# KeyuWu-CS/MonoHair

Measured on AMD Instinct MI355X. Metric: PMVO iterations/sec (60x1080p views, 256^3 volume), higher is better.
Workload: dtype f32

## Files before the change

monohair_amd/csrc/mh_key_blocks.h:

```cpp
template <int NI, int KN>
__device__ __forceinline__ void mh_key_block4(unsigned (&ke)[KN], unsigned (&ko)[KN], const float2 (&g)[4],
                                              const float (&DX)[KN], const float (&DY)[KN], int ib) {
    static_assert(NI >= 1 && NI <= 4 && NI <= KN, "mh_key_block4: 1..4 items");
    float a[NI], b[NI], c[NI];
    if constexpr (NI == 4) {
        asm volatile(
            "v_mul_f32_e32 %[a0], %[t0x], %[x0]\n\t"
            "v_mul_f32_e32 %[a1], %[t0x], %[x1]\n\t"
            "v_mul_f32_e32 %[a2], %[t0x], %[x2]\n\t"
            "v_mul_f32_e32 %[a3], %[t0x], %[x3]\n\t"
            "v_mul_f32_e32 %[b0], %[t0y], %[y0]\n\t"
            "v_mul_f32_e32 %[b1], %[t0y], %[y1]\n\t"
            "v_mul_f32_e32 %[b2], %[t0y], %[y2]\n\t"
            "v_mul_f32_e32 %[b3], %[t0y], %[y3]\n\t"
            "v_mul_f32_e32 %[c0], %[t2x], %[x0]\n\t"
            "v_mul_f32_e32 %[c1], %[t2x], %[x1]\n\t"
            "v_mul_f32_e32 %[c2], %[t2x], %[x2]\n\t"
            "v_mul_f32_e32 %[c3], %[t2x], %[x3]\n\t"
            "v_add_f32_e32 %[a0], %[a0], %[b0]\n\t"
            "v_add_f32_e32 %[a1], %[a1], %[b1]\n\t"
            "v_add_f32_e32 %[a2], %[a2], %[b2]\n\t"
            "v_add_f32_e32 %[a3], %[a3], %[b3]\n\t"
            "v_mul_f32_e32 %[b0], %[t2y], %[y0]\n\t"
            "v_mul_f32_e32 %[b1], %[t2y], %[y1]\n\t"
// ... 172 lines not shown
            "v_mul_f32_e32 %[b0], %[t1y], %[y0]\n\t"
            "v_mul_f32_e32 %[b1], %[t1y], %[y1]\n\t"
            "v_mul_f32_e32 %[c0], %[t3x], %[x0]\n\t"
            "v_mul_f32_e32 %[c1], %[t3x], %[x1]\n\t"
            "v_add_f32_e32 %[a0], %[a0], %[b0]\n\t"
            "v_add_f32_e32 %[a1], %[a1], %[b1]\n\t"
            "v_mul_f32_e32 %[b0], %[t3y], %[y0]\n\t"
            "v_mul_f32_e32 %[b1], %[t3y], %[y1]\n\t"
            "v_sub_f32_e64 %[a0], %[cc], |%[a0]|\n\t"
            "v_sub_f32_e64 %[a1], %[cc], |%[a1]|\n\t"
            "v_add_f32_e32 %[c0], %[c0], %[b0]\n\t"
            "v_add_f32_e32 %[c1], %[c1], %[b1]\n\t"
            "v_lshl_or_b32 %[a0], %[a0], 5, %[i0]\n\t"
            "v_lshl_or_b32 %[a1], %[a1], 5, %[i0]\n\t"
            "v_sub_f32_e64 %[c0], %[cc], |%[c0]|\n\t"
            "v_sub_f32_e64 %[c1], %[cc], |%[c1]|\n\t"
            "v_lshl_or_b32 %[c0], %[c0], 5, %[i1]\n\t"
            "v_lshl_or_b32 %[c1], %[c1], 5, %[i1]\n\t"
            "v_min3_u32 %[o0], %[o0], %[a0], %[c0]\n\t"
            "v_min3_u32 %[o1], %[o1], %[a1], %[c1]"
            : [e0] "+v"(ke[0]), [e1] "+v"(ke[1]), [o0] "+v"(ko[0]), [o1] "+v"(ko[1]), [a0] "=&v"(a[0]), [a1] "=&v"(a[1]), [b0] "=&v"(b[0]), [b1] "=&v"(b[1]), [c0] "=&v"(c[0]), [c1] "=&v"(c[1])
            : [t0x] "v"(g[0].x), [t0y] "v"(g[0].y), [t1x] "v"(g[1].x), [t1y] "v"(g[1].y), [t2x] "v"(g[2].x), [t2y] "v"(g[2].y), [t3x] "v"(g[3].x), [t3y] "v"(g[3].y), [x0] "v"(DX[0]), [y0] "v"(DY[0]), [x1] "v"(DX[1]), [y1] "v"(DY[1]), [cc] "s"(MH_KEY_C), [i0] "s"(ib), [i1] "s"(ib + 1)
            : "memory");
    }
    else if constexpr (NI == 1) {
        asm volatile(
            "v_mul_f32_e32 %[a0], %[t0x], %[x0]\n\t"
            "v_mul_f32_e32 %[b0], %[t0y], %[y0]\n\t"
            "v_mul_f32_e32 %[c0], %[t2x], %[x0]\n\t"
            "v_add_f32_e32 %[a0], %[a0], %[b0]\n\t"
            "v_mul_f32_e32 %[b0], %[t2y], %[y0]\n\t"
            "v_sub_f32_e64 %[a0], %[cc], |%[a0]|\n\t"
            "v_add_f32_e32 %[c0], %[c0], %[b0]\n\t"
            "v_lshl_or_b32 %[a0], %[a0], 5, %[i0]\n\t"
            "v_sub_f32_e64 %[c0], %[cc], |%[c0]|\n\t"
            "v_lshl_or_b32 %[c0], %[c0], 5, %[i1]\n\t"
            "v_min3_u32 %[e0], %[e0], %[a0], %[c0]\n\t"
            "v_mul_f32_e32 %[a0], %[t1x], %[x0]\n\t"
            "v_mul_f32_e32 %[b0], %[t1y], %[y0]\n\t"
            "v_mul_f32_e32 %[c0], %[t3x], %[x0]\n\t"
            "v_add_f32_e32 %[a0], %[a0], %[b0]\n\t"
            "v_mul_f32_e32 %[b0], %[t3y], %[y0]\n\t"
            "v_sub_f32_e64 %[a0], %[cc], |%[a0]|\n\t"
            "v_add_f32_e32 %[c0], %[c0], %[b0]\n\t"
            "v_lshl_or_b32 %[a0], %[a0], 5, %[i0]\n\t"
            "v_sub_f32_e64 %[c0], %[cc], |%[c0]|\n\t"
            "v_lshl_or_b32 %[c0], %[c0], 5, %[i1]\n\t"
            "v_min3_u32 %[o0], %[o0], %[a0], %[c0]"
            : [e0] "+v"(ke[0]), [o0] "+v"(ko[0]), [a0] "=&v"(a[0]), [b0] "=&v"(b[0]), [c0] "=&v"(c[0])
            : [t0x] "v"(g[0].x), [t0y] "v"(g[0].y), [t1x] "v"(g[1].x), [t1y] "v"(g[1].y), [t2x] "v"(g[2].x), [t2y] "v"(g[2].y), [t3x] "v"(g[3].x), [t3y] "v"(g[3].y), [x0] "v"(DX[0]), [y0] "v"(DY[0]), [cc] "s"(MH_KEY_C), [i0] "s"(ib), [i1] "s"(ib + 1)
            : "memory");
    }
}
```

monohair_amd/csrc/pmvo_search.hip:

```cpp
#include "mh_search_common.h"
#include "../../include/mh_pmvo_lab.h"

__device__ __forceinline__ void mh_sample_next(const float *__restrict__ cam, float X0, float X1, float X2,
                                               float ori_r, float ori_c, float Hf, float Wf, float off, float &S0,
                                               float &S1, float &S2, int forms) {
    alignas(16) float rec[16];
    mh_sample_rank(cam, X0, X1, X2, ori_r, ori_c, Hf, Wf, rec, forms);
    mh_sample_item(reinterpret_cast<const float4 *>(rec), off, S0, S1, S2);
}

__device__ __forceinline__ float mh_one_minus_abs(float x) {
    float r;
    asm("v_sub_f32_e64 %0, 1.0, |%1|" : "=v"(r) : "v"(x));
    return r;
}

template <int K, int T>
__global__ __launch_bounds__(T) void mh_search_kernel(MhViews vw, const float *__restrict__ offs, int S, int nrank,
                                                      int rank_step, const float *__restrict__ pts, int N, int P1,
                                                      float thr, const float *__restrict__ ori_c,
                                                      const int32_t *__restrict__ base_idx,
                                                      const float *__restrict__ base_val,
                                                      const float4 *__restrict__ taps, float *__restrict__ line_ori,
                                                      float *__restrict__ min_loss, uint8_t *__restrict__ high_conf,
// ... 182 lines not shown
        asm("v_cmp_lt_f32_e64 %[m0], %[l0], %[a0]\n\t"
            "v_cmp_lt_f32_e64 %[m1], %[l1], %[a1]\n\t"
            "v_cmp_lt_f32_e64 %[m2], %[l2], %[a2]\n\t"
            "v_cmp_lt_f32_e64 %[m3], %[l3], %[a3]\n\t"
            "v_cndmask_b32_e64 %[a0], %[a0], %[l0], %[m0]\n\t"
            "v_cndmask_b32_e64 %[a1], %[a1], %[l1], %[m1]\n\t"
            "v_cndmask_b32_e64 %[a2], %[a2], %[l2], %[m2]\n\t"
            "v_cndmask_b32_e64 %[a3], %[a3], %[l3], %[m3]\n\t"
            "v_cndmask_b32_e64 %[b0], %[b0], %[cf], %[m0]\n\t"
            "v_cndmask_b32_e64 %[b1], %[b1], %[cf], %[m1]\n\t"
            "v_cndmask_b32_e64 %[b2], %[b2], %[cf], %[m2]\n\t"
            "v_cndmask_b32_e64 %[b3], %[b3], %[cf], %[m3]"
            : [a0] "+v"(ML[0]), [a1] "+v"(ML[1]), [a2] "+v"(ML[2]), [a3] "+v"(ML[3]), [b0] "+v"(BC[0]),
              [b1] "+v"(BC[1]), [b2] "+v"(BC[2]), [b3] "+v"(BC[3]), [m0] "=&s"(m0), [m1] "=&s"(m1), [m2] "=&s"(m2),
              [m3] "=&s"(m3)
            : [l0] "v"(l[0]), [l1] "v"(l[1]), [l2] "v"(l[2]), [l3] "v"(l[3]), [cf] "v"(cf));
    } else if constexpr (KA == 3) {
        unsigned long long m0, m1, m2;
        asm("v_cmp_lt_f32_e64 %[m0], %[l0], %[a0]\n\t"
            "v_cmp_lt_f32_e64 %[m1], %[l1], %[a1]\n\t"
            "v_cmp_lt_f32_e64 %[m2], %[l2], %[a2]\n\t"
            "v_cndmask_b32_e64 %[a0], %[a0], %[l0], %[m0]\n\t"
            "v_cndmask_b32_e64 %[a1], %[a1], %[l1], %[m1]\n\t"
            "v_cndmask_b32_e64 %[a2], %[a2], %[l2], %[m2]\n\t"
            "v_cndmask_b32_e64 %[b0], %[b0], %[cf], %[m0]\n\t"
            "v_cndmask_b32_e64 %[b1], %[b1], %[cf], %[m1]\n\t"
            "v_cndmask_b32_e64 %[b2], %[b2], %[cf], %[m2]"
            : [a0] "+v"(ML[0]), [a1] "+v"(ML[1]), [a2] "+v"(ML[2]), [b0] "+v"(BC[0]), [b1] "+v"(BC[1]),
              [b2] "+v"(BC[2]), [m0] "=&s"(m0), [m1] "=&s"(m1), [m2] "=&s"(m2)
            : [l0] "v"(l[0]), [l1] "v"(l[1]), [l2] "v"(l[2]), [cf] "v"(cf));
    } else if constexpr (KA == 2) {
        unsigned long long m0, m1;
        asm("v_cmp_lt_f32_e64 %[m0], %[l0], %[a0]\n\t"
            "v_cmp_lt_f32_e64 %[m1], %[l1], %[a1]\n\t"
            "s_nop 0\n\t"
            "v_cndmask_b32_e64 %[a0], %[a0], %[l0], %[m0]\n\t"
            "v_cndmask_b32_e64 %[a1], %[a1], %[l1], %[m1]\n\t"
            "v_cndmask_b32_e64 %[b0], %[b0], %[cf], %[m0]\n\t"
            "v_cndmask_b32_e64 %[b1], %[b1], %[cf], %[m1]"
            : [a0] "+v"(ML[0]), [a1] "+v"(ML[1]), [b0] "+v"(BC[0]), [b1] "+v"(BC[1]), [m0] "=&s"(m0), [m1] "=&s"(m1)
            : [l0] "v"(l[0]), [l1] "v"(l[1]), [cf] "v"(cf));
    } else {
#pragma unroll
        for (int j = 0; j < KA; ++j) {
            const bool upd = l[j] < ML[j];
            ML[j] = upd ? l[j] : ML[j];
            BC[j] = upd ? cf : BC[j];
        }
    }
}

#define MH_KEY_C 1.00006103515625f
#define MH_KEY_E 6.103515625e-05f
#define MH_KEY_BAD 0xF0000000u
#ifndef MH_KEY_MIN_TAPS
#define MH_KEY_MIN_TAPS 10
#endif
#define MH_KEY_PAD 4
template <bool BIGP>
__device__ __forceinline__ int mh_key_walked(int c) {
    return (c - (BIGP ? 0 : 1) + MH_KEY_PAD - 1) & ~(MH_KEY_PAD - 1);
}
template <bool BIGP>
__device__ __forceinline__ int mh_key_staged(int c) {
    const int w = mh_key_walked<BIGP>(c);
    return w > c ? w : c;
}
__device__ unsigned long long mh_key_stats_dev[4];
extern "C" int mh_debug_key_stats(unsigned long long *out, int reset) {
    if (hipMemcpyFromSymbol(out, HIP_SYMBOL(mh_key_stats_dev), sizeof(unsigned long long) * 4) != hipSuccess) return -1;
    if (reset) {
        const unsigned long long z[4] = {0, 0, 0, 0};
        if (hipMemcpyToSymbol(HIP_SYMBOL(mh_key_stats_dev), z, sizeof(z)) != hipSuccess) return -1;
    }
    return 0;
}
#define MH_KEY_COUNT_ALWAYS(i) do { if ((tid & 63) == 0) atomicAdd(&mh_key_stats_dev[i], 1ull); } while (0)
#ifdef MH_KEY_STATS
#define MH_KEY_COUNT(i) MH_KEY_COUNT_ALWAYS(i)
#else
#define MH_KEY_COUNT(i) do { } while (0)
#endif
__device__ __forceinline__ unsigned mh_tap_key(float cs, int idx) {
    float t;
    unsigned k;
    asm("v_sub_f32_e64 %0, %2, |%1|" : "=v"(t) : "v"(cs), "s"(MH_KEY_C));
    asm("v_lshl_or_b32 %0, %1, 5, %2" : "=v"(k) : "v"(t), "s"(idx));
    return k;
}
__device__ __forceinline__ unsigned mh_min3u(unsigned a, unsigned b, unsigned c) {
    unsigned r;
    asm("v_min3_u32 %0, %1, %2, %3" : "=v"(r) : "v"(a), "v"(b), "v"(c));
    return r;
}

#include "mh_key_blocks.h"

#define MH_S3_GRP 4
#ifndef MH_S3_WAVES
#define MH_S3_WAVES 5
#endif
#ifndef MH_S3_WAVES_SELECT
#define MH_S3_WAVES_SELECT MH_S3_WAVES
#endif
#define MH_S3_CAP 1280

template <bool BIG>
struct MhCascS {
    float a0 = 0.0f, a1 = 0.0f, a2 = 0.0f;
    __device__ __forceinline__ void flush(int v) {
        a1 = a1 + a0;
        a0 = 0.0f;
        if constexpr (BIG) {
            if ((v & 0xF0) == 0) {
                a2 = a2 + a1;
                a1 = 0.0f;
            }
        }
    }
    __device__ __forceinline__ float done() const { return BIG ? (a0 + a1) + a2 : (a0 + a1); }
};

__device__ __forceinline__ int mh_wave_prefix_sum(int x) {
#define MH_DPP_ADD(CTRL, ROWS) x += __builtin_amdgcn_update_dpp(0, x, CTRL, ROWS, 0xF, false)
    MH_DPP_ADD(0x111, 0xF);
    MH_DPP_ADD(0x112, 0xF);
    MH_DPP_ADD(0x114, 0xF);
    MH_DPP_ADD(0x118, 0xF);
    MH_DPP_ADD(0x142, 0xA);
    MH_DPP_ADD(0x143, 0xC);
#undef MH_DPP_ADD
    return x;
}

__device__ __forceinline__ int mh_lane_now() {
    int lane;
    asm volatile("v_mbcnt_lo_u32_b32 %0, -1, 0\n\tv_mbcnt_hi_u32_b32 %0, -1, %0" : "=v"(lane));
    return lane;
}

// ... 186 lines not shown
                DX[2 * jp] = dx.x;
                DX[2 * jp + 1] = dx.y;
                DY[2 * jp] = dy.x;
                DY[2 * jp + 1] = dy.y;
            }
            if constexpr (KA & 1) {
                float row, col;
                mh_pixel_of_fast1(cam, X0[KA - 1], X1[KA - 1], X2[KA - 1], Hf, Wf, row, col);
                mh_unit2_fast1(row - hdr.z, col - hdr.w, DX[KA - 1], DY[KA - 1]);
            }
        }
        constexpr int GRP = MH_S3_GRP;
        auto select_body = [&]() {
#pragma unroll
            for (int j = 0; j < KA; ++j) {
                ML[j] = mh_one_minus_abs(mh_vadd(mh_vmul(t0.x, DX[j]), mh_vmul(t0.y, DY[j])));
                BC[j] = t0.z;
            }
            auto process = [&](const float4 (&g)[GRP], int t) {
#pragma unroll
                for (int u = 0; u < GRP; ++u) {
                    if (t + u < ntap) {
                        const float4 tp = g[u];
                        float l[KN];
#pragma unroll
                        for (int j = 0; j < KA; ++j)
                            l[j] = mh_one_minus_abs(mh_vadd(mh_vmul(tp.x, DX[j]), mh_vmul(tp.y, DY[j])));
                        mh_tap_update<KN>(ML, BC, l, tp.z);
                    }
                }
            };
            float4 ga[GRP], gb[GRP];
#pragma unroll
            for (int u = 0; u < GRP; ++u) ga[u] = rec[2 + u];
            for (int t = 1; t < ntap;) {
#pragma unroll
                for (int u = 0; u < GRP; ++u) gb[u] = rec[1 + t + GRP + u];
                process(ga, t);
                t += GRP;
                if (t >= ntap) break;
#pragma unroll
                for (int u = 0; u < GRP; ++u) ga[u] = rec[1 + t + GRP + u];
                process(gb, t);
                t += GRP;
            }
        };
        __builtin_amdgcn_s_setprio(0);
        if constexpr (!KEYS) {
            select_body();
        } else {
            bool again = (ntap <= MH_KEY_MIN_TAPS) || !(t0.x == t0.x && t0.y == t0.y);
            MH_KEY_COUNT(0);
            if (again) MH_KEY_COUNT(1);
            if (!again) {
                const int ntp = mh_key_walked<BIGP>(ntap);
                unsigned ke[KN], ko[KN];
                const unsigned rec1 = (unsigned)(size_t)(const __attribute__((address_space(3))) float4 *)(rec + 1);
                auto process = [&](const float2 (&g)[GRP], int t) {
                    const int ib = (t & 63) >> 1;
                    static_assert(MH_KEY_PAD == 4 && GRP == 4, "the key block takes four taps");
                    if constexpr (KM > 0) mh_key_block4<KM, KN>(ke, ko, g, DX, DY, ib);
                };
                auto group = [&](int ta, int tb) {
                    const float2 *__restrict__ t2 = reinterpret_cast<const float2 *>(rec + 1);
                    float2 ga[GRP], gb[GRP];
#pragma unroll
                    for (int u = 0; u < GRP; ++u) ga[u] = t2[2 * (ta + u)];
                    if constexpr (BIGP || KM == 0) {
#pragma unroll
                        for (int j = 0; j < KN; ++j) ke[j] = ko[j] = 0xFFFFFFFFu;
                    } else {
                        const int is = ntap - 1;
                        const float2 ts = t2[2 * is];
                        const bool even = (is & 1) == 0;
#pragma unroll
                        for (int j = 0; j < KM; ++j) {
                            const unsigned k = mh_tap_key(mh_vadd(mh_vmul(ts.x, DX[j]), mh_vmul(ts.y, DY[j])), is >> 1);
                            ke[j] = even ? k : 0xFFFFFFFFu;
                            ko[j] = even ? 0xFFFFFFFFu : k;
                        }
                    }
                    for (int t = ta; t < tb;) {
#pragma unroll
                        for (int u = 0; u < GRP; ++u) gb[u] = t2[2 * (t + GRP + u)];
                        process(ga, t);
                        t += GRP;
                        if (t >= tb) break;
#pragma unroll
                        for (int u = 0; u < GRP; ++u) ga[u] = t2[2 * (t + GRP + u)];
                        process(gb, t);
                        t += GRP;
                    }
                };
                unsigned best[KN], badr[KN];
                auto winner = [&](int ta, bool first) {
#pragma unroll
                    for (int j = 0; j < KM; ++j) {
                        const bool odd = ko[j] < ke[j];
                        const unsigned kb = odd ? ko[j] : ke[j];
                        const unsigned ad = rec1 + 16u * (unsigned)ta + ((kb & 31u) << 5) + (odd ? 16u : 0u);
                        const bool take = first || kb < (best[j] & ~31u);
                        best[j] = take ? kb : best[j];
                        badr[j] = take ? ad : badr[j];
                    }
                };
                if constexpr (!BIGP) {
                    group(0, ntp);
                    winner(0, true);
                } else {
                    group(0, ntp < 64 ? ntp : 64);
                    winner(0, true);
                    for (int ta = 64; ta < ntp; ta += 64) {
                        group(ta, ntp < ta + 64 ? ntp : ta + 64);
                        winner(ta, false);
                    }
                }
                unsigned worst = best[0];
#pragma unroll
                for (int j = 1; j < KM; ++j) worst = max(worst, best[j]);
                const bool bad = worst >= MH_KEY_BAD;
#pragma unroll
                for (int j = 0; j < KM; ++j) {
                    BC[j] = *reinterpret_cast<const __attribute__((address_space(3))) float *>((size_t)(badr[j] + 8u));
                    ML[j] = __uint_as_float(__builtin_amdgcn_alignbit(7u, best[j], 5u)) - MH_KEY_E;
                }
                again = __ballot(bad) != 0ull;
                if (again) MH_KEY_COUNT_ALWAYS(2);
            }
            if (again) select_body();
        }
        __builtin_amdgcn_s_setprio(1);
#pragma unroll
        for (int j = 0; j < KA; ++j) {
            const float w = BC[j];
            num[j].a0 = num[j].a0 + ML[j] * w;
            den[j].a0 = den[j].a0 + w;
            cnt[j] += (w > 0.0f) ? 1 : 0;
        }
    };
    const int lane = tid & 63, wave = __builtin_amdgcn_readfirstlane(tid >> 6);
    int c = c_first, pre = pre_first;
    for (int vb = 0; vb < V; vb += 64) {
        if (vb) {
            const int vv = vb + lane;
            c = (vv < V) ? (int)vcnt[(size_t)vv * N + n] : 0;
            pre = mh_wave_prefix_sum(mh_list_records<KEYS, BIGP>(c));
        }
        bool staged = vb == 0;
        unsigned long long todo = __ballot(c != 0);
        int base = 0;
        if constexpr (LEFT) {
            if (left && lane == 0) lf.vis[vb >> 6] = todo;
        }
        while (todo) {
            const unsigned long long take = todo & __ballot(pre - base <= MH_S3_CAP);
            if (!staged) {
                mh_stage_batch<T, KEYS, BIGP>(taps, s_taps, vb, n, N, P1, c, pre, base, take, wave);
                __syncthreads();
            }
            staged = false;
            if constexpr (KA > 0) {
                unsigned long long m = take;
                while (m) {
                    const int b = (int)__builtin_ctzll(m);
                    m &= m - 1;
                    flush_upto(vb + b);
                    const int cb = __builtin_amdgcn_readlane(c, b);
                    const int L = mh_list_records<KEYS, BIGP>(cb);
                    const int off = __builtin_amdgcn_readlane(pre, b) - L - base;
                    one_view(vb + b, s_taps + off, cb);
                }
            }
            if constexpr (LEFT) {
// ... 412 lines not shown
```

Measured before the change: 1812.

## Use block-index keys with a single min accumulator in the small-tap key search

After: 1833 (median of 6 runs). 1.2% higher.

```diff
diff --git a/monohair_amd/csrc/mh_key_blocks.h b/monohair_amd/csrc/mh_key_blocks.h
--- a/monohair_amd/csrc/mh_key_blocks.h
+++ b/monohair_amd/csrc/mh_key_blocks.h
@@ -248,3 +248,458 @@
             : "memory");
     }
 }
+
+template <int NI, int KN, bool FOLD>
+__device__ __forceinline__ void mh_key_blockm4(unsigned (&acc)[KN], unsigned (&kk)[KN], const float2 (&g)[4],
+                                               const float (&DX)[KN], const float (&DY)[KN], int ib) {
+    static_assert(NI >= 1 && NI <= 4 && NI <= KN, "mh_key_blockm4: 1..4 items");
+    constexpr int NW = NI < 2 ? NI : 2;
+    float a[NW], b[NW], c[NW];
+    [[maybe_unused]] float d[NW];
+    if constexpr (NI == 4) {
+        if constexpr (FOLD) {
+            asm volatile(
+                "v_mul_f32_e32 %[a0], %[t0x], %[x0]\n\t"
+                "v_mul_f32_e32 %[a1], %[t0x], %[x1]\n\t"
+                "v_mul_f32_e32 %[b0], %[t0y], %[y0]\n\t"
+                "v_mul_f32_e32 %[b1], %[t0y], %[y1]\n\t"
+                "v_mul_f32_e32 %[c0], %[t2x], %[x0]\n\t"
+                "v_mul_f32_e32 %[c1], %[t2x], %[x1]\n\t"
+                "v_add_f32_e32 %[a0], %[a0], %[b0]\n\t"
+                "v_add_f32_e32 %[a1], %[a1], %[b1]\n\t"
+                "v_mul_f32_e32 %[b0], %[t2y], %[y0]\n\t"
+                "v_mul_f32_e32 %[b1], %[t2y], %[y1]\n\t"
+                "v_sub_f32_e64 %[a0], %[cc], |%[a0]|\n\t"
+                "v_sub_f32_e64 %[a1], %[cc], |%[a1]|\n\t"
+                "v_add_f32_e32 %[c0], %[c0], %[b0]\n\t"
+                "v_add_f32_e32 %[c1], %[c1], %[b1]\n\t"
+                "v_mul_f32_e32 %[d0], %[t1x], %[x0]\n\t"
+                "v_mul_f32_e32 %[d1], %[t1x], %[x1]\n\t"
+                "v_sub_f32_e64 %[c0], %[cc], |%[c0]|\n\t"
+                "v_sub_f32_e64 %[c1], %[cc], |%[c1]|\n\t"
+                "v_mul_f32_e32 %[b0], %[t1y], %[y0]\n\t"
+                "v_mul_f32_e32 %[b1], %[t1y], %[y1]\n\t"
+                "v_min_u32_e32 %[a0], %[a0], %[c0]\n\t"
+                "v_min_u32_e32 %[a1], %[a1], %[c1]\n\t"
+                "v_mul_f32_e32 %[c0], %[t3x], %[x0]\n\t"
+                "v_mul_f32_e32 %[c1], %[t3x], %[x1]\n\t"
+                "v_add_f32_e32 %[d0], %[d0], %[b0]\n\t"
+                "v_add_f32_e32 %[d1], %[d1], %[b1]\n\t"
+                "v_mul_f32_e32 %[b0], %[t3y], %[y0]\n\t"
+                "v_mul_f32_e32 %[b1], %[t3y], %[y1]\n\t"
+                "v_sub_f32_e64 %[d0], %[cc], |%[d0]|\n\t"
+                "v_sub_f32_e64 %[d1], %[cc], |%[d1]|\n\t"
+                "v_add_f32_e32 %[c0], %[c0], %[b0]\n\t"
+                "v_add_f32_e32 %[c1], %[c1], %[b1]\n\t"
+                "v_sub_f32_e64 %[c0], %[cc], |%[c0]|\n\t"
+                "v_sub_f32_e64 %[c1], %[cc], |%[c1]|\n\t"
+                "v_min3_u32 %[a0], %[a0], %[d0], %[c0]\n\t"
+                "v_min3_u32 %[a1], %[a1], %[d1], %[c1]\n\t"
+                "v_lshl_or_b32 %[a0], %[a0], 4, %[ib]\n\t"
+                "v_lshl_or_b32 %[a1], %[a1], 4, %[ib]\n\t"
+                "v_min3_u32 %[m0], %[m0], %[k0], %[a0]\n\t"
+                "v_min3_u32 %[m1], %[m1], %[k1], %[a1]\n\t"
+                "v_mul_f32_e32 %[a0], %[t0x], %[x2]\n\t"
+                "v_mul_f32_e32 %[a1], %[t0x], %[x3]\n\t"
+                "v_mul_f32_e32 %[b0], %[t0y], %[y2]\n\t"
+                "v_mul_f32_e32 %[b1], %[t0y], %[y3]\n\t"
+                "v_mul_f32_e32 %[c0], %[t2x], %[x2]\n\t"
+                "v_mul_f32_e32 %[c1], %[t2x], %[x3]\n\t"
+                "v_add_f32_e32 %[a0], %[a0], %[b0]\n\t"
+                "v_add_f32_e32 %[a1], %[a1], %[b1]\n\t"
+                "v_mul_f32_e32 %[b0], %[t2y], %[y2]\n\t"
+                "v_mul_f32_e32 %[b1], %[t2y], %[y3]\n\t"
+                "v_sub_f32_e64 %[a0], %[cc], |%[a0]|\n\t"
+                "v_sub_f32_e64 %[a1], %[cc], |%[a1]|\n\t"
+                "v_add_f32_e32 %[c0], %[c0], %[b0]\n\t"
+                "v_add_f32_e32 %[c1], %[c1], %[b1]\n\t"
+                "v_mul_f32_e32 %[d0], %[t1x], %[x2]\n\t"
+                "v_mul_f32_e32 %[d1], %[t1x], %[x3]\n\t"
+                "v_sub_f32_e64 %[c0], %[cc], |%[c0]|\n\t"
+                "v_sub_f32_e64 %[c1], %[cc], |%[c1]|\n\t"
+                "v_mul_f32_e32 %[b0], %[t1y], %[y2]\n\t"
+                "v_mul_f32_e32 %[b1], %[t1y], %[y3]\n\t"
+                "v_min_u32_e32 %[a0], %[a0], %[c0]\n\t"
+                "v_min_u32_e32 %[a1], %[a1], %[c1]\n\t"
+                "v_mul_f32_e32 %[c0], %[t3x], %[x2]\n\t"
+                "v_mul_f32_e32 %[c1], %[t3x], %[x3]\n\t"
+                "v_add_f32_e32 %[d0], %[d0], %[b0]\n\t"
+                "v_add_f32_e32 %[d1], %[d1], %[b1]\n\t"
+                "v_mul_f32_e32 %[b0], %[t3y], %[y2]\n\t"
+                "v_mul_f32_e32 %[b1], %[t3y], %[y3]\n\t"
+                "v_sub_f32_e64 %[d0], %[cc], |%[d0]|\n\t"
+                "v_sub_f32_e64 %[d1], %[cc], |%[d1]|\n\t"
+                "v_add_f32_e32 %[c0], %[c0], %[b0]\n\t"
+                "v_add_f32_e32 %[c1], %[c1], %[b1]\n\t"
+                "v_sub_f32_e64 %[c0], %[cc], |%[c0]|\n\t"
+                "v_sub_f32_e64 %[c1], %[cc], |%[c1]|\n\t"
+                "v_min3_u32 %[a0], %[a0], %[d0], %[c0]\n\t"
+                "v_min3_u32 %[a1], %[a1], %[d1], %[c1]\n\t"
+                "v_lshl_or_b32 %[a0], %[a0], 4, %[ib]\n\t"
+                "v_lshl_or_b32 %[a1], %[a1], 4, %[ib]\n\t"
+                "v_min3_u32 %[m2], %[m2], %[k2], %[a0]\n\t"
+                "v_min3_u32 %[m3], %[m3], %[k3], %[a1]"
+                : [m0] "+v"(acc[0]), [m1] "+v"(acc[1]), [m2] "+v"(acc[2]), [m3] "+v"(acc[3]), [a0] "=&v"(a[0]), [a1] "=&v"(a[1]), [b0] "=&v"(b[0]), [b1] "=&v"(b[1]), [c0] "=&v"(c[0]), [c1] "=&v"(c[1]), [d0] "=&v"(d[0]), [d1] "=&v"(d[1])
+                : [t0x] "v"(g[0].x), [t0y] "v"(g[0].y), [t1x] "v"(g[1].x), [t1y] "v"(g[1].y), [t2x] "v"(g[2].x), [t2y] "v"(g[2].y), [t3x] "v"(g[3].x), [t3y] "v"(g[3].y), [x0] "v"(DX[0]), [y0] "v"(DY[0]), [x1] "v"(DX[1]), [y1] "v"(DY[1]), [x2] "v"(DX[2]), [y2] "v"(DY[2]), [x3] "v"(DX[3]), [y3] "v"(DY[3]), [k0] "v"(kk[0]), [k1] "v"(kk[1]), [k2] "v"(kk[2]), [k3] "v"(kk[3]), [cc] "s"(MH_KEY_C), [ib] "s"(ib)
+                : "memory");
+        }
+        else {
+            asm volatile(
+                "v_mul_f32_e32 %[a0], %[t0x], %[x0]\n\t"
+                "v_mul_f32_e32 %[a1], %[t0x], %[x1]\n\t"
+                "v_mul_f32_e32 %[b0], %[t0y], %[y0]\n\t"
+                "v_mul_f32_e32 %[b1], %[t0y], %[y1]\n\t"
+                "v_mul_f32_e32 %[c0], %[t2x], %[x0]\n\t"
+                "v_mul_f32_e32 %[c1], %[t2x], %[x1]\n\t"
+                "v_add_f32_e32 %[a0], %[a0], %[b0]\n\t"
+                "v_add_f32_e32 %[a1], %[a1], %[b1]\n\t"
+                "v_mul_f32_e32 %[b0], %[t2y], %[y0]\n\t"
+                "v_mul_f32_e32 %[b1], %[t2y], %[y1]\n\t"
+                "v_sub_f32_e64 %[a0], %[cc], |%[a0]|\n\t"
+                "v_sub_f32_e64 %[a1], %[cc], |%[a1]|\n\t"
+                "v_add_f32_e32 %[c0], %[c0], %[b0]\n\t"
+                "v_add_f32_e32 %[c1], %[c1], %[b1]\n\t"
+                "v_mul_f32_e32 %[k0], %[t1x], %[x0]\n\t"
+                "v_mul_f32_e32 %[k1], %[t1x], %[x1]\n\t"
+                "v_sub_f32_e64 %[c0], %[cc], |%[c0]|\n\t"
+                "v_sub_f32_e64 %[c1], %[cc], |%[c1]|\n\t"
+                "v_mul_f32_e32 %[b0], %[t1y], %[y0]\n\t"
+                "v_mul_f32_e32 %[b1], %[t1y], %[y1]\n\t"
+                "v_min_u32_e32 %[a0], %[a0], %[c0]\n\t"
+                "v_min_u32_e32 %[a1], %[a1], %[c1]\n\t"
+                "v_mul_f32_e32 %[c0], %[t3x], %[x0]\n\t"
+                "v_mul_f32_e32 %[c1], %[t3x], %[x1]\n\t"
+                "v_add_f32_e32 %[k0], %[k0], %[b0]\n\t"
+                "v_add_f32_e32 %[k1], %[k1], %[b1]\n\t"
+                "v_mul_f32_e32 %[b0], %[t3y], %[y0]\n\t"
+                "v_mul_f32_e32 %[b1], %[t3y], %[y1]\n\t"
+                "v_sub_f32_e64 %[k0], %[cc], |%[k0]|\n\t"
+                "v_sub_f32_e64 %[k1], %[cc], |%[k1]|\n\t"
+                "v_add_f32_e32 %[c0], %[c0], %[b0]\n\t"
+                "v_add_f32_e32 %[c1], %[c1], %[b1]\n\t"
+                "v_sub_f32_e64 %[c0], %[cc], |%[c0]|\n\t"
+                "v_sub_f32_e64 %[c1], %[cc], |%[c1]|\n\t"
+                "v_min3_u32 %[a0], %[a0], %[k0], %[c0]\n\t"
+                "v_min3_u32 %[a1], %[a1], %[k1], %[c1]\n\t"
+                "v_lshl_or_b32 %[k0], %[a0], 4, %[ib]\n\t"
+                "v_lshl_or_b32 %[k1], %[a1], 4, %[ib]\n\t"
+                "v_mul_f32_e32 %[a0], %[t0x], %[x2]\n\t"
+                "v_mul_f32_e32 %[a1], %[t0x], %[x3]\n\t"
+                "v_mul_f32_e32 %[b0], %[t0y], %[y2]\n\t"
+                "v_mul_f32_e32 %[b1], %[t0y], %[y3]\n\t"
+                "v_mul_f32_e32 %[c0], %[t2x], %[x2]\n\t"
+                "v_mul_f32_e32 %[c1], %[t2x], %[x3]\n\t"
+                "v_add_f32_e32 %[a0], %[a0], %[b0]\n\t"
+                "v_add_f32_e32 %[a1], %[a1], %[b1]\n\t"
+                "v_mul_f32_e32 %[b0], %[t2y], %[y2]\n\t"
+                "v_mul_f32_e32 %[b1], %[t2y], %[y3]\n\t"
+                "v_sub_f32_e64 %[a0], %[cc], |%[a0]|\n\t"
+                "v_sub_f32_e64 %[a1], %[cc], |%[a1]|\n\t"
+                "v_add_f32_e32 %[c0], %[c0], %[b0]\n\t"
+                "v_add_f32_e32 %[c1], %[c1], %[b1]\n\t"
+                "v_mul_f32_e32 %[k2], %[t1x], %[x2]\n\t"
+                "v_mul_f32_e32 %[k3], %[t1x], %[x3]\n\t"
+                "v_sub_f32_e64 %[c0], %[cc], |%[c0]|\n\t"
+                "v_sub_f32_e64 %[c1], %[cc], |%[c1]|\n\t"
+                "v_mul_f32_e32 %[b0], %[t1y], %[y2]\n\t"
+                "v_mul_f32_e32 %[b1], %[t1y], %[y3]\n\t"
+                "v_min_u32_e32 %[a0], %[a0], %[c0]\n\t"
+                "v_min_u32_e32 %[a1], %[a1], %[c1]\n\t"
+                "v_mul_f32_e32 %[c0], %[t3x], %[x2]\n\t"
+                "v_mul_f32_e32 %[c1], %[t3x], %[x3]\n\t"
+                "v_add_f32_e32 %[k2], %[k2], %[b0]\n\t"
+                "v_add_f32_e32 %[k3], %[k3], %[b1]\n\t"
+                "v_mul_f32_e32 %[b0], %[t3y], %[y2]\n\t"
+                "v_mul_f32_e32 %[b1], %[t3y], %[y3]\n\t"
+                "v_sub_f32_e64 %[k2], %[cc], |%[k2]|\n\t"
+                "v_sub_f32_e64 %[k3], %[cc], |%[k3]|\n\t"
+                "v_add_f32_e32 %[c0], %[c0], %[b0]\n\t"
+                "v_add_f32_e32 %[c1], %[c1], %[b1]\n\t"
+                "v_sub_f32_e64 %[c0], %[cc], |%[c0]|\n\t"
+                "v_sub_f32_e64 %[c1], %[cc], |%[c1]|\n\t"
+                "v_min3_u32 %[a0], %[a0], %[k2], %[c0]\n\t"
+                "v_min3_u32 %[a1], %[a1], %[k3], %[c1]\n\t"
+                "v_lshl_or_b32 %[k2], %[a0], 4, %[ib]\n\t"
+                "v_lshl_or_b32 %[k3], %[a1], 4, %[ib]"
+                : [k0] "=&v"(kk[0]), [k1] "=&v"(kk[1]), [k2] "=&v"(kk[2]), [k3] "=&v"(kk[3]), [a0] "=&v"(a[0]), [a1] "=&v"(a[1]), [b0] "=&v"(b[0]), [b1] "=&v"(b[1]), [c0] "=&v"(c[0]), [c1] "=&v"(c[1])
+                : [t0x] "v"(g[0].x), [t0y] "v"(g[0].y), [t1x] "v"(g[1].x), [t1y] "v"(g[1].y), [t2x] "v"(g[2].x), [t2y] "v"(g[2].y), [t3x] "v"(g[3].x), [t3y] "v"(g[3].y), [x0] "v"(DX[0]), [y0] "v"(DY[0]), [x1] "v"(DX[1]), [y1] "v"(DY[1]), [x2] "v"(DX[2]), [y2] "v"(DY[2]), [x3] "v"(DX[3]), [y3] "v"(DY[3]), [cc] "s"(MH_KEY_C), [ib] "s"(ib)
+                : "memory");
+        }
+    }
+    else if constexpr (NI == 3) {
+        if constexpr (FOLD) {
+            asm volatile(
+                "v_mul_f32_e32 %[a0], %[t0x], %[x0]\n\t"
+                "v_mul_f32_e32 %[a1], %[t0x], %[x1]\n\t"
+                "v_mul_f32_e32 %[b0], %[t0y], %[y0]\n\t"
+                "v_mul_f32_e32 %[b1], %[t0y], %[y1]\n\t"
+                "v_mul_f32_e32 %[c0], %[t2x], %[x0]\n\t"
+                "v_mul_f32_e32 %[c1], %[t2x], %[x1]\n\t"
+                "v_add_f32_e32 %[a0], %[a0], %[b0]\n\t"
+                "v_add_f32_e32 %[a1], %[a1], %[b1]\n\t"
+                "v_mul_f32_e32 %[b0], %[t2y], %[y0]\n\t"
+                "v_mul_f32_e32 %[b1], %[t2y], %[y1]\n\t"
+                "v_sub_f32_e64 %[a0], %[cc], |%[a0]|\n\t"
+                "v_sub_f32_e64 %[a1], %[cc], |%[a1]|\n\t"
+                "v_add_f32_e32 %[c0], %[c0], %[b0]\n\t"
+                "v_add_f32_e32 %[c1], %[c1], %[b1]\n\t"
+                "v_mul_f32_e32 %[d0], %[t1x], %[x0]\n\t"
+                "v_mul_f32_e32 %[d1], %[t1x], %[x1]\n\t"
+                "v_sub_f32_e64 %[c0], %[cc], |%[c0]|\n\t"
+                "v_sub_f32_e64 %[c1], %[cc], |%[c1]|\n\t"
+                "v_mul_f32_e32 %[b0], %[t1y], %[y0]\n\t"
+                "v_mul_f32_e32 %[b1], %[t1y], %[y1]\n\t"
+                "v_min_u32_e32 %[a0], %[a0], %[c0]\n\t"
+                "v_min_u32_e32 %[a1], %[a1], %[c1]\n\t"
+                "v_mul_f32_e32 %[c0], %[t3x], %[x0]\n\t"
+                "v_mul_f32_e32 %[c1], %[t3x], %[x1]\n\t"
+                "v_add_f32_e32 %[d0], %[d0], %[b0]\n\t"
+                "v_add_f32_e32 %[d1], %[d1], %[b1]\n\t"
+                "v_mul_f32_e32 %[b0], %[t3y], %[y0]\n\t"
+                "v_mul_f32_e32 %[b1], %[t3y], %[y1]\n\t"
+                "v_sub_f32_e64 %[d0], %[cc], |%[d0]|\n\t"
+                "v_sub_f32_e64 %[d1], %[cc], |%[d1]|\n\t"
+                "v_add_f32_e32 %[c0], %[c0], %[b0]\n\t"
+                "v_add_f32_e32 %[c1], %[c1], %[b1]\n\t"
+                "v_sub_f32_e64 %[c0], %[cc], |%[c0]|\n\t"
+                "v_sub_f32_e64 %[c1], %[cc], |%[c1]|\n\t"
+                "v_min3_u32 %[a0], %[a0], %[d0], %[c0]\n\t"
+                "v_min3_u32 %[a1], %[a1], %[d1], %[c1]\n\t"
+                "v_lshl_or_b32 %[a0], %[a0], 4, %[ib]\n\t"
+                "v_lshl_or_b32 %[a1], %[a1], 4, %[ib]\n\t"
+                "v_min3_u32 %[m0], %[m0], %[k0], %[a0]\n\t"
+                "v_min3_u32 %[m1], %[m1], %[k1], %[a1]\n\t"
+                "v_mul_f32_e32 %[a0], %[t0x], %[x2]\n\t"
+                "v_mul_f32_e32 %[b0], %[t0y], %[y2]\n\t"
+                "v_mul_f32_e32 %[c0], %[t2x], %[x2]\n\t"
+                "v_add_f32_e32 %[a0], %[a0], %[b0]\n\t"
+                "v_mul_f32_e32 %[b0], %[t2y], %[y2]\n\t"
+                "v_sub_f32_e64 %[a0], %[cc], |%[a0]|\n\t"
+                "v_add_f32_e32 %[c0], %[c0], %[b0]\n\t"
+                "v_mul_f32_e32 %[d0], %[t1x], %[x2]\n\t"
+                "v_sub_f32_e64 %[c0], %[cc], |%[c0]|\n\t"
+                "v_mul_f32_e32 %[b0], %[t1y], %[y2]\n\t"
+                "v_min_u32_e32 %[a0], %[a0], %[c0]\n\t"
+                "v_mul_f32_e32 %[c0], %[t3x], %[x2]\n\t"
+                "v_add_f32_e32 %[d0], %[d0], %[b0]\n\t"
+                "v_mul_f32_e32 %[b0], %[t3y], %[y2]\n\t"
+                "v_sub_f32_e64 %[d0], %[cc], |%[d0]|\n\t"
+                "v_add_f32_e32 %[c0], %[c0], %[b0]\n\t"
+                "v_sub_f32_e64 %[c0], %[cc], |%[c0]|\n\t"
+                "v_min3_u32 %[a0], %[a0], %[d0], %[c0]\n\t"
+                "v_lshl_or_b32 %[a0], %[a0], 4, %[ib]\n\t"
+                "v_min3_u32 %[m2], %[m2], %[k2], %[a0]"
+                : [m0] "+v"(acc[0]), [m1] "+v"(acc[1]), [m2] "+v"(acc[2]), [a0] "=&v"(a[0]), [a1] "=&v"(a[1]), [b0] "=&v"(b[0]), [b1] "=&v"(b[1]), [c0] "=&v"(c[0]), [c1] "=&v"(c[1]), [d0] "=&v"(d[0]), [d1] "=&v"(d[1])
+                : [t0x] "v"(g[0].x), [t0y] "v"(g[0].y), [t1x] "v"(g[1].x), [t1y] "v"(g[1].y), [t2x] "v"(g[2].x), [t2y] "v"(g[2].y), [t3x] "v"(g[3].x), [t3y] "v"(g[3].y), [x0] "v"(DX[0]), [y0] "v"(DY[0]), [x1] "v"(DX[1]), [y1] "v"(DY[1]), [x2] "v"(DX[2]), [y2] "v"(DY[2]), [k0] "v"(kk[0]), [k1] "v"(kk[1]), [k2] "v"(kk[2]), [cc] "s"(MH_KEY_C), [ib] "s"(ib)
+                : "memory");
+        }
+        else {
+            asm volatile(
+                "v_mul_f32_e32 %[a0], %[t0x], %[x0]\n\t"
+                "v_mul_f32_e32 %[a1], %[t0x], %[x1]\n\t"
+                "v_mul_f32_e32 %[b0], %[t0y], %[y0]\n\t"
+                "v_mul_f32_e32 %[b1], %[t0y], %[y1]\n\t"
+                "v_mul_f32_e32 %[c0], %[t2x], %[x0]\n\t"
+                "v_mul_f32_e32 %[c1], %[t2x], %[x1]\n\t"
+                "v_add_f32_e32 %[a0], %[a0], %[b0]\n\t"
+                "v_add_f32_e32 %[a1], %[a1], %[b1]\n\t"
+                "v_mul_f32_e32 %[b0], %[t2y], %[y0]\n\t"
+                "v_mul_f32_e32 %[b1], %[t2y], %[y1]\n\t"
+                "v_sub_f32_e64 %[a0], %[cc], |%[a0]|\n\t"
+                "v_sub_f32_e64 %[a1], %[cc], |%[a1]|\n\t"
+                "v_add_f32_e32 %[c0], %[c0], %[b0]\n\t"
+                "v_add_f32_e32 %[c1], %[c1], %[b1]\n\t"
+                "v_mul_f32_e32 %[k0], %[t1x], %[x0]\n\t"
+                "v_mul_f32_e32 %[k1], %[t1x], %[x1]\n\t"
+                "v_sub_f32_e64 %[c0], %[cc], |%[c0]|\n\t"
+                "v_sub_f32_e64 %[c1], %[cc], |%[c1]|\n\t"
+                "v_mul_f32_e32 %[b0], %[t1y], %[y0]\n\t"
+                "v_mul_f32_e32 %[b1], %[t1y], %[y1]\n\t"
+                "v_min_u32_e32 %[a0], %[a0], %[c0]\n\t"
+                "v_min_u32_e32 %[a1], %[a1], %[c1]\n\t"
+                "v_mul_f32_e32 %[c0], %[t3x], %[x0]\n\t"
+                "v_mul_f32_e32 %[c1], %[t3x], %[x1]\n\t"
+                "v_add_f32_e32 %[k0], %[k0], %[b0]\n\t"
+                "v_add_f32_e32 %[k1], %[k1], %[b1]\n\t"
+                "v_mul_f32_e32 %[b0], %[t3y], %[y0]\n\t"
+                "v_mul_f32_e32 %[b1], %[t3y], %[y1]\n\t"
+                "v_sub_f32_e64 %[k0], %[cc], |%[k0]|\n\t"
+                "v_sub_f32_e64 %[k1], %[cc], |%[k1]|\n\t"
+                "v_add_f32_e32 %[c0], %[c0], %[b0]\n\t"
+                "v_add_f32_e32 %[c1], %[c1], %[b1]\n\t"
+                "v_sub_f32_e64 %[c0], %[cc], |%[c0]|\n\t"
+                "v_sub_f32_e64 %[c1], %[cc], |%[c1]|\n\t"
+                "v_min3_u32 %[a0], %[a0], %[k0], %[c0]\n\t"
+                "v_min3_u32 %[a1], %[a1], %[k1], %[c1]\n\t"
+                "v_lshl_or_b32 %[k0], %[a0], 4, %[ib]\n\t"
+                "v_lshl_or_b32 %[k1], %[a1], 4, %[ib]\n\t"
+                "v_mul_f32_e32 %[a0], %[t0x], %[x2]\n\t"
+                "v_mul_f32_e32 %[b0], %[t0y], %[y2]\n\t"
+                "v_mul_f32_e32 %[c0], %[t2x], %[x2]\n\t"
+                "v_add_f32_e32 %[a0], %[a0], %[b0]\n\t"
+                "v_mul_f32_e32 %[b0], %[t2y], %[y2]\n\t"
+                "v_sub_f32_e64 %[a0], %[cc], |%[a0]|\n\t"
+                "v_add_f32_e32 %[c0], %[c0], %[b0]\n\t"
+                "v_mul_f32_e32 %[k2], %[t1x], %[x2]\n\t"
+                "v_sub_f32_e64 %[c0], %[cc], |%[c0]|\n\t"
+                "v_mul_f32_e32 %[b0], %[t1y], %[y2]\n\t"
+                "v_min_u32_e32 %[a0], %[a0], %[c0]\n\t"
+                "v_mul_f32_e32 %[c0], %[t3x], %[x2]\n\t"
+                "v_add_f32_e32 %[k2], %[k2], %[b0]\n\t"
+                "v_mul_f32_e32 %[b0], %[t3y], %[y2]\n\t"
+                "v_sub_f32_e64 %[k2], %[cc], |%[k2]|\n\t"
+                "v_add_f32_e32 %[c0], %[c0], %[b0]\n\t"
+                "v_sub_f32_e64 %[c0], %[cc], |%[c0]|\n\t"
+                "v_min3_u32 %[a0], %[a0], %[k2], %[c0]\n\t"
+                "v_lshl_or_b32 %[k2], %[a0], 4, %[ib]"
+                : [k0] "=&v"(kk[0]), [k1] "=&v"(kk[1]), [k2] "=&v"(kk[2]), [a0] "=&v"(a[0]), [a1] "=&v"(a[1]), [b0] "=&v"(b[0]), [b1] "=&v"(b[1]), [c0] "=&v"(c[0]), [c1] "=&v"(c[1])
+                : [t0x] "v"(g[0].x), [t0y] "v"(g[0].y), [t1x] "v"(g[1].x), [t1y] "v"(g[1].y), [t2x] "v"(g[2].x), [t2y] "v"(g[2].y), [t3x] "v"(g[3].x), [t3y] "v"(g[3].y), [x0] "v"(DX[0]), [y0] "v"(DY[0]), [x1] "v"(DX[1]), [y1] "v"(DY[1]), [x2] "v"(DX[2]), [y2] "v"(DY[2]), [cc] "s"(MH_KEY_C), [ib] "s"(ib)
+                : "memory");
+        }
+    }
+    else if constexpr (NI == 2) {
+        if constexpr (FOLD) {
+            asm volatile(
+                "v_mul_f32_e32 %[a0], %[t0x], %[x0]\n\t"
+                "v_mul_f32_e32 %[a1], %[t0x], %[x1]\n\t"
+                "v_mul_f32_e32 %[b0], %[t0y], %[y0]\n\t"
+                "v_mul_f32_e32 %[b1], %[t0y], %[y1]\n\t"
+                "v_mul_f32_e32 %[c0], %[t2x], %[x0]\n\t"
+                "v_mul_f32_e32 %[c1], %[t2x], %[x1]\n\t"
+                "v_add_f32_e32 %[a0], %[a0], %[b0]\n\t"
+                "v_add_f32_e32 %[a1], %[a1], %[b1]\n\t"
+                "v_mul_f32_e32 %[b0], %[t2y], %[y0]\n\t"
+                "v_mul_f32_e32 %[b1], %[t2y], %[y1]\n\t"
+                "v_sub_f32_e64 %[a0], %[cc], |%[a0]|\n\t"
+                "v_sub_f32_e64 %[a1], %[cc], |%[a1]|\n\t"
+                "v_add_f32_e32 %[c0], %[c0], %[b0]\n\t"
+                "v_add_f32_e32 %[c1], %[c1], %[b1]\n\t"
+                "v_mul_f32_e32 %[d0], %[t1x], %[x0]\n\t"
+                "v_mul_f32_e32 %[d1], %[t1x], %[x1]\n\t"
+                "v_sub_f32_e64 %[c0], %[cc], |%[c0]|\n\t"
+                "v_sub_f32_e64 %[c1], %[cc], |%[c1]|\n\t"
+                "v_mul_f32_e32 %[b0], %[t1y], %[y0]\n\t"
+                "v_mul_f32_e32 %[b1], %[t1y], %[y1]\n\t"
+                "v_min_u32_e32 %[a0], %[a0], %[c0]\n\t"
+                "v_min_u32_e32 %[a1], %[a1], %[c1]\n\t"
+                "v_mul_f32_e32 %[c0], %[t3x], %[x0]\n\t"
+                "v_mul_f32_e32 %[c1], %[t3x], %[x1]\n\t"
+                "v_add_f32_e32 %[d0], %[d0], %[b0]\n\t"
+                "v_add_f32_e32 %[d1], %[d1], %[b1]\n\t"
+                "v_mul_f32_e32 %[b0], %[t3y], %[y0]\n\t"
+                "v_mul_f32_e32 %[b1], %[t3y], %[y1]\n\t"
+                "v_sub_f32_e64 %[d0], %[cc], |%[d0]|\n\t"
+                "v_sub_f32_e64 %[d1], %[cc], |%[d1]|\n\t"
+                "v_add_f32_e32 %[c0], %[c0], %[b0]\n\t"
+                "v_add_f32_e32 %[c1], %[c1], %[b1]\n\t"
+                "v_sub_f32_e64 %[c0], %[cc], |%[c0]|\n\t"
+                "v_sub_f32_e64 %[c1], %[cc], |%[c1]|\n\t"
+                "v_min3_u32 %[a0], %[a0], %[d0], %[c0]\n\t"
+                "v_min3_u32 %[a1], %[a1], %[d1], %[c1]\n\t"
+                "v_lshl_or_b32 %[a0], %[a0], 4, %[ib]\n\t"
+                "v_lshl_or_b32 %[a1], %[a1], 4, %[ib]\n\t"
+                "v_min3_u32 %[m0], %[m0], %[k0], %[a0]\n\t"
+                "v_min3_u32 %[m1], %[m1], %[k1], %[a1]"
+                : [m0] "+v"(acc[0]), [m1] "+v"(acc[1]), [a0] "=&v"(a[0]), [a1] "=&v"(a[1]), [b0] "=&v"(b[0]), [b1] "=&v"(b[1]), [c0] "=&v"(c[0]), [c1] "=&v"(c[1]), [d0] "=&v"(d[0]), [d1] "=&v"(d[1])
+                : [t0x] "v"(g[0].x), [t0y] "v"(g[0].y), [t1x] "v"(g[1].x), [t1y] "v"(g[1].y), [t2x] "v"(g[2].x), [t2y] "v"(g[2].y), [t3x] "v"(g[3].x), [t3y] "v"(g[3].y), [x0] "v"(DX[0]), [y0] "v"(DY[0]), [x1] "v"(DX[1]), [y1] "v"(DY[1]), [k0] "v"(kk[0]), [k1] "v"(kk[1]), [cc] "s"(MH_KEY_C), [ib] "s"(ib)
+                : "memory");
+        }
+        else {
+            asm volatile(
+                "v_mul_f32_e32 %[a0], %[t0x], %[x0]\n\t"
+                "v_mul_f32_e32 %[a1], %[t0x], %[x1]\n\t"
+                "v_mul_f32_e32 %[b0], %[t0y], %[y0]\n\t"
+                "v_mul_f32_e32 %[b1], %[t0y], %[y1]\n\t"
+                "v_mul_f32_e32 %[c0], %[t2x], %[x0]\n\t"
+                "v_mul_f32_e32 %[c1], %[t2x], %[x1]\n\t"
+                "v_add_f32_e32 %[a0], %[a0], %[b0]\n\t"
+                "v_add_f32_e32 %[a1], %[a1], %[b1]\n\t"
+                "v_mul_f32_e32 %[b0], %[t2y], %[y0]\n\t"
+                "v_mul_f32_e32 %[b1], %[t2y], %[y1]\n\t"
+                "v_sub_f32_e64 %[a0], %[cc], |%[a0]|\n\t"
+                "v_sub_f32_e64 %[a1], %[cc], |%[a1]|\n\t"
+                "v_add_f32_e32 %[c0], %[c0], %[b0]\n\t"
+                "v_add_f32_e32 %[c1], %[c1], %[b1]\n\t"
+                "v_mul_f32_e32 %[k0], %[t1x], %[x0]\n\t"
+                "v_mul_f32_e32 %[k1], %[t1x], %[x1]\n\t"
+                "v_sub_f32_e64 %[c0], %[cc], |%[c0]|\n\t"
+                "v_sub_f32_e64 %[c1], %[cc], |%[c1]|\n\t"
+                "v_mul_f32_e32 %[b0], %[t1y], %[y0]\n\t"
+                "v_mul_f32_e32 %[b1], %[t1y], %[y1]\n\t"
+                "v_min_u32_e32 %[a0], %[a0], %[c0]\n\t"
+                "v_min_u32_e32 %[a1], %[a1], %[c1]\n\t"
+                "v_mul_f32_e32 %[c0], %[t3x], %[x0]\n\t"
+                "v_mul_f32_e32 %[c1], %[t3x], %[x1]\n\t"
+                "v_add_f32_e32 %[k0], %[k0], %[b0]\n\t"
+                "v_add_f32_e32 %[k1], %[k1], %[b1]\n\t"
+                "v_mul_f32_e32 %[b0], %[t3y], %[y0]\n\t"
+                "v_mul_f32_e32 %[b1], %[t3y], %[y1]\n\t"
+                "v_sub_f32_e64 %[k0], %[cc], |%[k0]|\n\t"
+                "v_sub_f32_e64 %[k1], %[cc], |%[k1]|\n\t"
+                "v_add_f32_e32 %[c0], %[c0], %[b0]\n\t"
+                "v_add_f32_e32 %[c1], %[c1], %[b1]\n\t"
+                "v_sub_f32_e64 %[c0], %[cc], |%[c0]|\n\t"
+                "v_sub_f32_e64 %[c1], %[cc], |%[c1]|\n\t"
+                "v_min3_u32 %[a0], %[a0], %[k0], %[c0]\n\t"
+                "v_min3_u32 %[a1], %[a1], %[k1], %[c1]\n\t"
+                "v_lshl_or_b32 %[k0], %[a0], 4, %[ib]\n\t"
+                "v_lshl_or_b32 %[k1], %[a1], 4, %[ib]"
+                : [k0] "=&v"(kk[0]), [k1] "=&v"(kk[1]), [a0] "=&v"(a[0]), [a1] "=&v"(a[1]), [b0] "=&v"(b[0]), [b1] "=&v"(b[1]), [c0] "=&v"(c[0]), [c1] "=&v"(c[1])
+                : [t0x] "v"(g[0].x), [t0y] "v"(g[0].y), [t1x] "v"(g[1].x), [t1y] "v"(g[1].y), [t2x] "v"(g[2].x), [t2y] "v"(g[2].y), [t3x] "v"(g[3].x), [t3y] "v"(g[3].y), [x0] "v"(DX[0]), [y0] "v"(DY[0]), [x1] "v"(DX[1]), [y1] "v"(DY[1]), [cc] "s"(MH_KEY_C), [ib] "s"(ib)
+                : "memory");
+        }
+    }
+    else if constexpr (NI == 1) {
+        if constexpr (FOLD) {
+            asm volatile(
+                "v_mul_f32_e32 %[a0], %[t0x], %[x0]\n\t"
+                "v_mul_f32_e32 %[b0], %[t0y], %[y0]\n\t"
+                "v_mul_f32_e32 %[c0], %[t2x], %[x0]\n\t"
+                "v_add_f32_e32 %[a0], %[a0], %[b0]\n\t"
+                "v_mul_f32_e32 %[b0], %[t2y], %[y0]\n\t"
+                "v_sub_f32_e64 %[a0], %[cc], |%[a0]|\n\t"
+                "v_add_f32_e32 %[c0], %[c0], %[b0]\n\t"
+                "v_mul_f32_e32 %[d0], %[t1x], %[x0]\n\t"
+                "v_sub_f32_e64 %[c0], %[cc], |%[c0]|\n\t"
+                "v_mul_f32_e32 %[b0], %[t1y], %[y0]\n\t"
+                "v_min_u32_e32 %[a0], %[a0], %[c0]\n\t"
+                "v_mul_f32_e32 %[c0], %[t3x], %[x0]\n\t"
+                "v_add_f32_e32 %[d0], %[d0], %[b0]\n\t"
+                "v_mul_f32_e32 %[b0], %[t3y], %[y0]\n\t"
+                "v_sub_f32_e64 %[d0], %[cc], |%[d0]|\n\t"
+                "v_add_f32_e32 %[c0], %[c0], %[b0]\n\t"
+                "v_sub_f32_e64 %[c0], %[cc], |%[c0]|\n\t"
+                "v_min3_u32 %[a0], %[a0], %[d0], %[c0]\n\t"
+                "v_lshl_or_b32 %[a0], %[a0], 4, %[ib]\n\t"
+                "v_min3_u32 %[m0], %[m0], %[k0], %[a0]"
+                : [m0] "+v"(acc[0]), [a0] "=&v"(a[0]), [b0] "=&v"(b[0]), [c0] "=&v"(c[0]), [d0] "=&v"(d[0])
+                : [t0x] "v"(g[0].x), [t0y] "v"(g[0].y), [t1x] "v"(g[1].x), [t1y] "v"(g[1].y), [t2x] "v"(g[2].x), [t2y] "v"(g[2].y), [t3x] "v"(g[3].x), [t3y] "v"(g[3].y), [x0] "v"(DX[0]), [y0] "v"(DY[0]), [k0] "v"(kk[0]), [cc] "s"(MH_KEY_C), [ib] "s"(ib)
+                : "memory");
+        }
+        else {
+            asm volatile(
+                "v_mul_f32_e32 %[a0], %[t0x], %[x0]\n\t"
+                "v_mul_f32_e32 %[b0], %[t0y], %[y0]\n\t"
+                "v_mul_f32_e32 %[c0], %[t2x], %[x0]\n\t"
+                "v_add_f32_e32 %[a0], %[a0], %[b0]\n\t"
+                "v_mul_f32_e32 %[b0], %[t2y], %[y0]\n\t"
+                "v_sub_f32_e64 %[a0], %[cc], |%[a0]|\n\t"
+                "v_add_f32_e32 %[c0], %[c0], %[b0]\n\t"
+                "v_mul_f32_e32 %[k0], %[t1x], %[x0]\n\t"
+                "v_sub_f32_e64 %[c0], %[cc], |%[c0]|\n\t"
+                "v_mul_f32_e32 %[b0], %[t1y], %[y0]\n\t"
+                "v_min_u32_e32 %[a0], %[a0], %[c0]\n\t"
+                "v_mul_f32_e32 %[c0], %[t3x], %[x0]\n\t"
+                "v_add_f32_e32 %[k0], %[k0], %[b0]\n\t"
+                "v_mul_f32_e32 %[b0], %[t3y], %[y0]\n\t"
+                "v_sub_f32_e64 %[k0], %[cc], |%[k0]|\n\t"
+                "v_add_f32_e32 %[c0], %[c0], %[b0]\n\t"
+                "v_sub_f32_e64 %[c0], %[cc], |%[c0]|\n\t"
+                "v_min3_u32 %[a0], %[a0], %[k0], %[c0]\n\t"
+                "v_lshl_or_b32 %[k0], %[a0], 4, %[ib]"
+                : [k0] "=&v"(kk[0]), [a0] "=&v"(a[0]), [b0] "=&v"(b[0]), [c0] "=&v"(c[0])
+                : [t0x] "v"(g[0].x), [t0y] "v"(g[0].y), [t1x] "v"(g[1].x), [t1y] "v"(g[1].y), [t2x] "v"(g[2].x), [t2y] "v"(g[2].y), [t3x] "v"(g[3].x), [t3y] "v"(g[3].y), [x0] "v"(DX[0]), [y0] "v"(DY[0]), [cc] "s"(MH_KEY_C), [ib] "s"(ib)
+                : "memory");
+        }
+    }
+}
diff --git a/monohair_amd/csrc/pmvo_search.hip b/monohair_amd/csrc/pmvo_search.hip
--- a/monohair_amd/csrc/pmvo_search.hip
+++ b/monohair_amd/csrc/pmvo_search.hip
@@ -258,7 +258,8 @@
 
 #define MH_KEY_C 1.00006103515625f
 #define MH_KEY_E 6.103515625e-05f
-#define MH_KEY_BAD 0xF0000000u
+#define MH_KEY_BAD 0xF8000000u
+#define MH_KEY_BAD_TAP 0xF0000000u
 #ifndef MH_KEY_MIN_TAPS
 #define MH_KEY_MIN_TAPS 10
 #endif
@@ -287,11 +288,15 @@
 #else
 #define MH_KEY_COUNT(i) do { } while (0)
 #endif
-__device__ __forceinline__ unsigned mh_tap_key(float cs, int idx) {
+__device__ __forceinline__ float mh_key_tprime(float cs) {
     float t;
+    asm("v_sub_f32_e64 %0, %2, |%1|" : "=v"(t) : "v"(cs), "s"(MH_KEY_C));
+    return t;
+}
+__device__ __forceinline__ unsigned mh_seed_key(float cs, int blk) {
+    const float t = mh_key_tprime(cs);
     unsigned k;
-    asm("v_sub_f32_e64 %0, %2, |%1|" : "=v"(t) : "v"(cs), "s"(MH_KEY_C));
-    asm("v_lshl_or_b32 %0, %1, 5, %2" : "=v"(k) : "v"(t), "s"(idx));
+    asm("v_lshl_or_b32 %0, %1, 4, %2" : "=v"(k) : "v"(t), "s"(blk));
     return k;
 }
 __device__ __forceinline__ unsigned mh_min3u(unsigned a, unsigned b, unsigned c) {
@@ -584,7 +589,73 @@
             bool again = (ntap <= MH_KEY_MIN_TAPS) || !(t0.x == t0.x && t0.y == t0.y);
             MH_KEY_COUNT(0);
             if (again) MH_KEY_COUNT(1);
-            if (!again) {
+            if constexpr (!BIGP) {
+              if (!again) {
+                const int ntp = mh_key_walked<false>(ntap);
+                unsigned acc[KN], kk[KN];
+                const unsigned rec1 = (unsigned)(size_t)(const __attribute__((address_space(3))) float4 *)(rec + 1);
+                static_assert(MH_KEY_PAD == 4 && GRP == 4, "the key block takes four taps");
+                {
+                    const float2 *__restrict__ t2 = reinterpret_cast<const float2 *>(rec + 1);
+                    float2 ga[GRP], gb[GRP];
+#pragma unroll
+                    for (int u = 0; u < GRP; ++u) ga[u] = t2[2 * u];
+                    const int is = ntap - 1;
+                    const float2 ts = t2[2 * is];
+#pragma unroll
+                    for (int j = 0; j < KM; ++j)
+                        acc[j] = mh_seed_key(mh_vadd(mh_vmul(ts.x, DX[j]), mh_vmul(ts.y, DY[j])), is >> 2);
+                    for (int t = 0; t < ntp;) {
+#pragma unroll
+                        for (int u = 0; u < GRP; ++u) gb[u] = t2[2 * (t + GRP + u)];
+                        if constexpr (KM > 0) mh_key_blockm4<KM, KN, false>(acc, kk, ga, DX, DY, t >> 2);
+                        t += GRP;
+                        if (t >= ntp) {
+#pragma unroll
+                            for (int j = 0; j < KM; ++j) acc[j] = min(acc[j], kk[j]);
+                            break;
+                        }
+#pragma unroll
+                        for (int u = 0; u < GRP; ++u) ga[u] = t2[2 * (t + GRP + u)];
+                        if constexpr (KM > 0) mh_key_blockm4<KM, KN, true>(acc, kk, gb, DX, DY, t >> 2);
+                        t += GRP;
+                    }
+                }
+                unsigned worst = acc[0];
+#pragma unroll
+                for (int j = 1; j < KM; ++j) worst = max(worst, acc[j]);
+                const bool bad = worst >= MH_KEY_BAD;
+                typedef const __attribute__((address_space(3))) mh_v2f *lds_f2;
+                typedef const __attribute__((address_space(3))) float *lds_f1;
+#pragma unroll
+                for (int j0 = 0; j0 < KM; j0 += 2) {
+                    if (j0) __builtin_amdgcn_sched_barrier(0);
+                    unsigned ad[2], mb[2];
+                    mh_v2f w[2][3];
+#pragma unroll
+                    for (int j = j0; j < KM && j < j0 + 2; ++j) {
+                        ad[j - j0] = rec1 + ((acc[j] & 15u) << 6);
+                        mb[j - j0] = __builtin_amdgcn_alignbit(3u, acc[j], 4u);
+#pragma unroll
+                        for (int u = 0; u < 3; ++u) w[j - j0][u] = *reinterpret_cast<lds_f2>((size_t)(ad[j - j0] + 16u * u));
+                    }
+#pragma unroll
+                    for (int j = j0; j < KM && j < j0 + 2; ++j) {
+                        unsigned off = 56u;
+#pragma unroll
+                        for (int u = 2; u >= 0; --u) {
+                            const mh_v2f tp = w[j - j0][u];
+                            const float tq = mh_key_tprime(mh_vadd(mh_vmul(tp.x, DX[j]), mh_vmul(tp.y, DY[j])));
+                            off = (__float_as_uint(tq) == mb[j - j0]) ? 8u + 16u * u : off;
+                        }
+                        BC[j] = *reinterpret_cast<lds_f1>((size_t)(ad[j - j0] + off));
+                        ML[j] = __uint_as_float(mb[j - j0]) - MH_KEY_E;
+                    }
+                }
+                again = __ballot(bad) != 0ull;
+                if (again) MH_KEY_COUNT_ALWAYS(2);
+              }
+            } else if (!again) {
                 const int ntp = mh_key_walked<BIGP>(ntap);
                 unsigned ke[KN], ko[KN];
                 const unsigned rec1 = (unsigned)(size_t)(const __attribute__((address_space(3))) float4 *)(rec + 1);
@@ -598,20 +669,8 @@
                     float2 ga[GRP], gb[GRP];
 #pragma unroll
                     for (int u = 0; u < GRP; ++u) ga[u] = t2[2 * (ta + u)];
-                    if constexpr (BIGP || KM == 0) {
-#pragma unroll
-                        for (int j = 0; j < KN; ++j) ke[j] = ko[j] = 0xFFFFFFFFu;
-                    } else {
-                        const int is = ntap - 1;
-                        const float2 ts = t2[2 * is];
-                        const bool even = (is & 1) == 0;
-#pragma unroll
-                        for (int j = 0; j < KM; ++j) {
-                            const unsigned k = mh_tap_key(mh_vadd(mh_vmul(ts.x, DX[j]), mh_vmul(ts.y, DY[j])), is >> 1);
-                            ke[j] = even ? k : 0xFFFFFFFFu;
-                            ko[j] = even ? 0xFFFFFFFFu : k;
-                        }
-                    }
+#pragma unroll
+                    for (int j = 0; j < KN; ++j) ke[j] = ko[j] = 0xFFFFFFFFu;
                     for (int t = ta; t < tb;) {
 #pragma unroll
                         for (int u = 0; u < GRP; ++u) gb[u] = t2[2 * (t + GRP + u)];
@@ -636,21 +695,16 @@
                         badr[j] = take ? ad : badr[j];
                     }
                 };
-                if constexpr (!BIGP) {
-                    group(0, ntp);
-                    winner(0, true);
-                } else {
-                    group(0, ntp < 64 ? ntp : 64);
-                    winner(0, true);
-                    for (int ta = 64; ta < ntp; ta += 64) {
-                        group(ta, ntp < ta + 64 ? ntp : ta + 64);
-                        winner(ta, false);
-                    }
+                group(0, ntp < 64 ? ntp : 64);
+                winner(0, true);
+                for (int ta = 64; ta < ntp; ta += 64) {
+                    group(ta, ntp < ta + 64 ? ntp : ta + 64);
+                    winner(ta, false);
                 }
                 unsigned worst = best[0];
 #pragma unroll
                 for (int j = 1; j < KM; ++j) worst = max(worst, best[j]);
-                const bool bad = worst >= MH_KEY_BAD;
+                const bool bad = worst >= MH_KEY_BAD_TAP;
 #pragma unroll
                 for (int j = 0; j < KM; ++j) {
                     BC[j] = *reinterpret_cast<const __attribute__((address_space(3))) float *>((size_t)(badr[j] + 8u));
```
